# nomadkaraoke/python-audio-separator

Measured on AMD Instinct MI355X. Metric: audio-sec separated / wall-sec (RTF), UVR-MDX-NET 44.1kHz stereo, 1/2/4/8 GPU, higher is better.
Workload: dtype f32 (I/O and accumulators; matrix products on the 16-bit pipe from block-scaled two-part fp16 operands, 22-bit products -- see arithmetic; fp32-exact setting timed in arithmetic_ab)

## Files before the change

python-audio-separator_amd/csrc/asx.hip:

```cpp
#include <hip/hip_runtime.h>

#include <algorithm>
#include <atomic>
#include <cmath>
#include <cstdarg>
#include <cstdio>
#include <cstdlib>
#include <cstring>
#include <functional>
#include <map>
#include <string>
#include <mutex>
#include <vector>

#include "../../include/asx.h"
#include "knobs.h"
#include "resample_plan.h"
#include "flac_dec_plan.h"

static void grant_lds(const void *kernel, int bytes) {
  static std::mutex mu;
  static std::map<const void *, int> granted;
  std::lock_guard<std::mutex> lock(mu);
  int &g = granted[kernel];
// ... 24 lines not shown
#include "kernels_hd.h"
#include "kernels_vr.h"
#include "kernels_ens.h"
#include "kernels_resample.h"
#include "kernels_flac.h"
#include "kernels_pcm_encode.h"
#include "kernels_flac_dec.h"

using namespace asx;

#include "engine_core.h"
#include "engine_mdx.h"

static int opt_nonneg(int32_t v) { return v < 0 ? 0 : (int)v; }
static int opt_onoff(int32_t v) { return v > 0 ? 1 : 0; }

static const struct EngineOption {
  const char *key;
  int asx_engine::*field;
  int EngineKnobs::*knob;
  int (*norm)(int32_t);
  const char *refusal = nullptr;
  int shipped = 0;
} kOptions[] = {
    {"winograd", &asx_engine::winograd, &EngineKnobs::winograd, opt_nonneg,
     "asx_set_option: winograd = %d names a superseded kernel generation that only an experimental build carries "
     "(python build.py --experimental); this library has 0 (direct kernel) and 3 (the default)", 3},
    {"winograd_stationary", &asx_engine::winos, &EngineKnobs::winos, opt_nonneg,
     "asx_set_option: the weight-stationary Winograd kernel (measured slower) is in experimental builds only (python build.py --experimental)"},
    {"winograd_bf16x6", &asx_engine::wino6, &EngineKnobs::wino6, opt_nonneg},
    {"gemm_bf16x6", &asx_engine::gemm_bf16x6, &EngineKnobs::gemm_bf16x6, opt_onoff},
    {"gemm_f16x3", &asx_engine::gemm_f16x3, &EngineKnobs::gemm_f16x3, opt_onoff},
    {"conv_direct_f16x3", &asx_engine::conv3h, &EngineKnobs::conv3h, opt_nonneg},
    {"conv_fuse_input", &asx_engine::conv_fuse_input, &EngineKnobs::conv_fuse_input, opt_onoff},
    {"tdf_fuse_output", &asx_engine::tdf_fuse_output, &EngineKnobs::tdf_fuse_output, opt_onoff},
    {"conv3h_partial_scratch", &asx_engine::conv3h_ps, &EngineKnobs::conv3h_ps, opt_onoff},
    {"conv3h_walk", &asx_engine::conv3h_walk, &EngineKnobs::conv3h_walk, opt_onoff},
    {"conv3h_tiled", &asx_engine::conv3h_tiled, &EngineKnobs::conv3h_tiled, opt_onoff},
    {"conv3h_merge_out", &asx_engine::conv3h_merge, &EngineKnobs::conv3h_merge, opt_nonneg},
    {"conv_down_bf16x6", &asx_engine::down6, &EngineKnobs::down6, opt_onoff},
    {"conv_up_bf16x6", &asx_engine::up6, &EngineKnobs::up6, opt_onoff},
    {"gemm_pair_images", &asx_engine::pair_images, &EngineKnobs::pair_images, opt_onoff,
     "asx_set_option: gemm_pair_images = 1 needs an experimental build (python build.py --experimental): the pair-image reader measured no "
     "faster in the nets and is not in the default library"},
};

static const EngineOption *find_option(const char *fn, const char *key) {
  for (const EngineOption &o : kOptions)
    if (!strcmp(key, o.key)) return &o;
  set_err("%s: unknown option '%s'", fn, key);
  return nullptr;
}

extern "C" {
// ... 1414 lines not shown

int asx_op_conv(asx_engine *e, const char *op, const float *x_host, int32_t B, int32_t cin, int32_t t, int32_t f,
                const float *w_host, const float *b_host, int32_t cout, const float *aux_host, int32_t relu,
                float *y_host) {
  REQUIRE(e && op && x_host && w_host && y_host && B > 0 && cin > 0 && cout > 0 && t > 0 && f > 0,
          "asx_op_conv: bad argument");
  HIPCHK(hipSetDevice(e->device));
  int kind;
  int to = t, fo = f;
  ConvView view;
  if (!strcmp(op, "conv3x3")) kind = CK_3X3;
  else if (!strcmp(op, "conv3x3_to_tiled") || !strcmp(op, "conv3x3_tiled") || !strcmp(op, "conv3x3_from_tiled")) {
    kind = CK_3X3;
    view.x_tiled = strcmp(op, "conv3x3_to_tiled") != 0;
    view.y_tiled = strcmp(op, "conv3x3_from_tiled") != 0;
  } else if (!strcmp(op, "down")) {
    kind = CK_DOWN;
    to = t / 2;
    fo = f / 2;
  } else if (!strcmp(op, "conv1x1")) kind = CK_1X1;
  else if (!strcmp(op, "up")) {
    kind = CK_UP;
    to = 2 * t;
    fo = 2 * f;
    REQUIRE(aux_host, "asx_op_conv(up): skip tensor required");
  } else {
    set_err("asx_op_conv: unknown op '%s'", op);
    return ASX_ERR_INVALID;
  }
  ConvLayer L;
  DevBuf dx, dy, dskip;
  BufGuard g{{&dx, &dy, &dskip, &L.w, &L.b, &L.wu, &L.wu2, &L.wu3, &L.wus, &L.wu6, &L.wu6h, &L.w3h, &L.wd6, &L.wup6}};
  CHK(conv_setup(L, kind, cin, cout, relu ? 1 : 0));
  CHK(conv_pack(L, w_host, b_host, e->winograd));
  CHK(to_dev(dx, x_host, (size_t)B * cin * t * f));
  const size_t ny = (size_t)B * cout * to * fo;
  CHK(dy.ensure(ny * 4));
// ... 1231 lines not shown
}

int asx_counter(const asx_engine *e, const char *name, int64_t *out) {
  REQUIRE(e && name && out, "asx_counter: null argument");
  const std::string nm(name);
  if (nm == "tdf3_launches") *out = (int64_t)g_tdf3_launches.load();
  else if (nm == "tdf3h_launches") *out = (int64_t)g_tdf3h_launches.load();
  else if (nm == "attn6_launches") *out = (int64_t)g_attn6_launches.load();
  else if (nm == "attn6h_launches") *out = (int64_t)g_attn6h_launches.load();
  else if (nm == "tdf3_gather_launches") *out = (int64_t)g_tdf3_gather_launches.load();
  else if (nm == "wino6_launches") *out = (int64_t)g_wino6_launches.load();
  else if (nm == "wino6h_launches") *out = (int64_t)g_wino6h_launches.load();
  else if (nm == "conv3h_launches") *out = (int64_t)g_conv3h_launches.load();
  else if (nm == "conv3h_fin_launches") *out = (int64_t)g_conv3h_fin_launches.load();
  else if (nm == "conv3h_tiled_launches") *out = (int64_t)g_conv3h_tiled_launches.load();
  else if (nm == "conv3h_merged_dispatches") *out = (int64_t)g_conv3h_merged_dispatches.load();
  else if (nm == "tdf_fused_output_launches") *out = (int64_t)g_tdf_fused_output_launches.load();
  else if (nm == "tdf3_pair_image_launches") *out = (int64_t)g_tdf3ps_launches.load();
  else if (nm == "down6_launches") *out = (int64_t)g_down6_launches.load();
  else if (nm == "up6_launches") *out = (int64_t)g_up6_launches.load();
  else if (nm == "hd_rounds") *out = (int64_t)g_hd_rounds.load();
  else if (nm == "vr_net_passes") *out = (int64_t)g_vr_net_passes.load();
  else if (nm == "v3_net_passes") *out = (int64_t)g_v3_net_passes.load();
  else if (nm == "rof_net_passes") *out = (int64_t)g_rof_net_passes.load();
  else if (nm == "flac_block_cycles") *out = (int64_t)e->flac_block_cycles;
  else if (nm == "flac_crc16_cycles") *out = (int64_t)e->flac_crc16_cycles;
  else {
    set_err("asx_counter: unknown counter '%s'", name);
    return ASX_ERR_INVALID;
  }
  return ASX_OK;
}

int asx_debug_trace(uint64_t *host, int64_t n_u64) {
  REQUIRE(host && n_u64 > 0 && n_u64 <= 4096 * 8, "asx_debug_trace: bad argument");
// ... 263 lines not shown
```

python-audio-separator_amd/csrc/engine_core.h:

```cpp
#pragma once

static thread_local char g_err[512] = "";
static void set_err(const char *fmt, ...) {
  va_list ap;
  va_start(ap, fmt);
  vsnprintf(g_err, sizeof(g_err), fmt, ap);
  va_end(ap);
}
#define HIPCHK(x)                                                                       \
  do {                                                                                  \
    hipError_t e_ = (x);                                                                \
    if (e_ != hipSuccess) {                                                             \
      set_err("%s:%d %s -> %s", __FILE__, __LINE__, #x, hipGetErrorString(e_));         \
      return ASX_ERR_HIP;                                                               \
    }                                                                                   \
  } while (0)
#define CHK(x)                    \
  do {                            \
    int r_ = (x);                 \
    if (r_ != ASX_OK) return r_;  \
  } while (0)
#define REQUIRE(cond, ...)        \
  do {                            \
    if (!(cond)) {                \
// ... 191 lines not shown
  std::vector<RsTable *> rs_tabs;
  std::mutex rs_mu;
  hipEvent_t div_ev = nullptr;
  hipStream_t div_stream = nullptr;
  std::vector<DevBuf> skip;
  int winograd = 3;
  int winos = 0;
  int gemm_bf16x6 = 1;
  int gemm_f16x3 = 1;
  int wino6 = 144;
  int conv3h = 144;
  int conv3h_ps = 1;
  int conv3h_walk = 1;
  int conv3h_tiled = 1;
  int conv3h_merge = 144;
  int conv_fuse_input = 1;
  int tdf_fuse_output = 1;
  int down6 = 1;
  int up6 = 1;
  int pair_images = 0;
  std::vector<W3Entry> w3;
  std::mutex w3_mu;
  bool prof = false;
  int prof_nprod = 0;
  std::vector<ProfRec> recs;
};

static int pick_batch(const asx_engine *e) { return e->cfg.max_batch > 0 ? e->cfg.max_batch : 64; }

#include "batching.h"
// ... 75 lines not shown
```

python-audio-separator_amd/csrc/engine_mdx.h:

```cpp
#pragma once

template <class CFG>
static void launch_conv_t(const ConvArgs &a, int nblk, hipStream_t s) {
  grant_lds(&conv_mfma_kernel<CFG>, CFG::LDS_BYTES);
  hipLaunchKernelGGL(conv_mfma_kernel<CFG>, dim3(nblk), dim3(256), CFG::LDS_BYTES, s, a);
}

static int conv_tile_h(int kind) { return kind == CK_UP ? 4 : 8; }

static int pick_nrep_conv(int cout) {
  const int ct = (cout + 15) / 16;
  int best = 1, best_pad = 1 << 30;
  for (int n = 3; n >= 1; --n) {
    const int pad = ((ct + n - 1) / n) * n - ct;
    if (pad < best_pad) {
      best_pad = pad;
      best = n;
    }
  }
  return best;
}
static int pick_nrep_up(int cout) {
  const int ct = (cout + 15) / 16;
  if (knobs().up_nrep == 4 && (4 * ct) % 4 == 0) return 4;
// ... 188 lines not shown
  HIPCHK(hipMemcpy(L.b.p, bp.data(), bp.size() * 4, hipMemcpyHostToDevice));
  return ASX_OK;
}

template <class CFG>
static void launch_conv_dma_t(const ConvArgs &a, int nblk, hipStream_t s) {
  grant_lds(&conv_dma_kernel<CFG>, CFG::LDS_BYTES);
  hipLaunchKernelGGL(conv_dma_kernel<CFG>, dim3(nblk), dim3(256), CFG::LDS_BYTES, s, a);
}

static std::atomic<long long> g_wino6_launches{0};
static std::atomic<long long> g_wino6h_launches{0};
static std::atomic<long long> g_conv3h_launches{0};
static std::atomic<long long> g_conv3h_fin_launches{0};
static std::atomic<long long> g_conv3h_tiled_launches{0};
static std::atomic<long long> g_conv3h_merged_dispatches{0};
static std::atomic<long long> g_down6_launches{0};
static std::atomic<long long> g_up6_launches{0};

struct ConvView {
  int64_t x_bstride = 0;
  int64_t y_bstride = 0;
  const float *res = nullptr;
  int64_t aux_bstride = 0;
  int act = -1;
  float alpha = 1.f;
  const ConvLayer *fin = nullptr;
  const float *fin_x = nullptr;
  bool x_tiled = false, y_tiled = false;
};

static bool conv3h_takes(const asx_engine *e, const ConvLayer &L, bool dma, const float *res, int act, int T, int F, int64_t y_bstride, const float *y) {
#ifdef ASX_EXPERIMENTAL_KERNELS
  if (e->winos == 1 && L.wus.p != nullptr) return false;
#endif
  return L.kind == CK_3X3 && e->winograd == 3 && e->gemm_bf16x6 > 0 && e->gemm_f16x3 > 0 && e->conv3h > 0 && L.cin <= e->conv3h && L.w3h.p != nullptr && dma &&
         res == nullptr && (act == ACT_RELU || act == ACT_NONE) && F % 32 == 0 && (int64_t)Conv3hCfg::C * T * F < ((int64_t)1 << 29) &&
         y_bstride % 4 == 0 && (reinterpret_cast<uintptr_t>(y) & 15) == 0;
}

static bool conv3h_tiled_ok(const asx_engine *e, const ConvLayer &L, int T) { return T % 4 == 0 && (L.cin == Conv3hCfg::C || e->conv3h_ps > 0); }

static size_t conv3h_ps_need(const ConvLayer &L, int B, int T, int F) {
  if (L.kind != CK_3X3 || L.w3h.p == nullptr || L.cin <= Conv3hCfg::C || F % 32 != 0 || B <= 0 || T <= 0) return 0;
  return (size_t)(L.cin / Conv3hCfg::C) * (size_t)Conv3hCfg::ps_bytes(B, (T + 3) / 4, F / 32);
}

static const Conv3hWalkTab *conv3h_walk_find(const asx_engine *e, int B, int tilesT, int tilesF, int mode, int nob) {
  for (const Conv3hWalkTab *t : e->c3h_walks)
    if (t->B == B && t->tilesT == tilesT && t->tilesF == tilesF && t->mode == mode && t->nob == nob) return t;
  return nullptr;
}
static int conv3h_walk_ensure(asx_engine *e, const ConvLayer &L, int B, int T, int F) {
  if (L.kind != CK_3X3 || L.w3h.p == nullptr || F % 32 != 0 || B <= 0 || T <= 0) return ASX_OK;
  const int tilesT = (T + 3) / 4, tilesF = F / 32, nb = L.cin / Conv3hCfg::C;
  for (int k = 0; k < (nb > 1 ? 4 : 2); ++k) {
// ... 65 lines not shown
  a.aux_bstride = v.aux_bstride ? v.aux_bstride : (int64_t)L.cout * out_plane;
  const int th = conv_tile_h(L.kind);
  a.tilesT = (a.To + th - 1) / th;
  a.tilesF = (a.Fo + 63) / 64;
  const int nblk = a.CG * a.tilesT * a.tilesF * B;
  if (nblk <= 0) return ASX_OK;
  const double outpix = (double)B * a.To * a.Fo;
  const double flops = 2.0 * taps * L.cin * L.cout * outpix;
  double bytes = 4.0 * ((double)B * L.cin * T * F + (double)L.cout * outpix * (L.kind == CK_UP ? 4 : 1));
  if (L.kind == CK_UP && skip) bytes += 4.0 * (double)L.cout * outpix * 4;
  if (v.res) bytes += 4.0 * (double)L.cout * outpix;
  int bad = 0;
  const bool dma = (F % 4 == 0) && ((reinterpret_cast<uintptr_t>(v.fin ? v.fin_x : x) & 15) == 0) && (a.x_bstride % 4 == 0) && !knobs().no_dma;
  REQUIRE(!v.fin || (v.fin->w1f.p != nullptr && L.cin == Conv3hCfg::C && conv3h_takes(e, L, dma, v.res, a.act, T, F, a.y_bstride, y)),
          "fused-input 3x3 conv: the layer does not run conv3h_kernel");
  REQUIRE(!(v.x_tiled || v.y_tiled) || (conv3h_takes(e, L, dma, v.res, a.act, T, F, a.y_bstride, y) && conv3h_tiled_ok(e, L, T) && !(v.x_tiled && v.fin)),
          "tile-order 3x3 conv: the layer does not run conv3h_kernel in a form that has the layout");
  const ConvArgs &d = a;
#ifdef ASX_EXPERIMENTAL_KERNELS
  if (L.kind == CK_3X3 && e->winograd == 3 && e->winos == 1 && dma && L.wus.p != nullptr && a.Fo % 32 == 0 && v.res == nullptr &&
      (a.act == ACT_RELU || a.act == ACT_NONE) && (int64_t)L.cin * T * F < ((int64_t)1 << 30)) {
    ConvArgs wa = a;
    wa.wp = L.wus.f();
    wa.CG = L.wu_cg;
    wa.tilesF = a.Fo / 32;
    const int NS = (a.To + 1) / 2;
    const int base = wa.CG * wa.tilesF * B;
    int RB = std::max(1, std::min((NS + 7) / 8, (2048 + base - 1) / base));
    const int SPB = (NS + RB - 1) / RB;
    RB = (NS + SPB - 1) / SPB;
    wa.tilesT = RB;
// ... 40 lines not shown
        grant_lds(kern, Conv3hCfg::LDS_BYTES);
        hipLaunchKernelGGL(kern, dim3(256), dim3(512), Conv3hCfg::LDS_BYTES, s, ca);
      };
      if constexpr (FIN) {
        if (yt) one(&conv3h_kernel<0, false, true, 0, false, true>);
        else one(&conv3h_kernel<0, false, true>);
      } else if constexpr ((PS & 2) != 0) {
        if (v.x_tiled) one(&conv3h_kernel<0, false, false, PS, true, false>);
        else one(&conv3h_kernel<0, false, false, PS>);
      } else {
        if (v.x_tiled && yt) one(&conv3h_kernel<0, false, false, PS, true, true>);
        else if (v.x_tiled) one(&conv3h_kernel<0, false, false, PS, true, false>);
        else if (yt) one(&conv3h_kernel<0, false, false, PS, false, true>);
        else one(&conv3h_kernel<0, false, false, PS>);
      }
      if (v.x_tiled || yt) g_conv3h_tiled_launches.fetch_add(ca.nob);
    };
    const int64_t plane = (int64_t)T * F;
    const int64_t ps_item = Conv3hCfg::ps_item_bytes(tilesT, tilesF);
    REQUIRE(!ps || (ps_item < ((int64_t)1 << 32) && e->c3h_ps.p != nullptr && e->c3h_ps.bytes >= conv3h_ps_need(L, B, T, F)),
            "conv3h_kernel: the partial-sum scratch is not sized for %d x %d x %d (the workspace set-up sizes it)", B, T, F);
    Conv3hArgs walk{};
    walk.B = B;
    walk.T = T;
    walk.F = F;
    walk.x_bstride = a.x_bstride;
    walk.y_bstride = a.y_bstride;
    walk.tilesT = tilesT;
    walk.tilesF = tilesF;
    walk.bw = wt->bw;
    walk.walk = reinterpret_cast<const u32x4 *>(wt->tab.p);
// ... 121 lines not shown
  }
  if (L.kind == CK_3X3 && e->winograd == 1 && dma && L.wu.p != nullptr) {
    ConvArgs wa = a;
    wa.wp = L.wu.f();
    wa.CG = L.wu_cg;
    wa.NCI = L.wu_nci;
    wa.tilesT = (a.To + WinoCfg::TH - 1) / WinoCfg::TH;
    wa.tilesF = (a.Fo + WinoCfg::TW - 1) / WinoCfg::TW;
    const int nb = wa.CG * wa.tilesT * wa.tilesF * B;
    grant_lds(&conv_wino_kernel, WinoCfg::LDS_BYTES);
    return timed(e, cls, flops, bytes, s, [&]() {
      hipLaunchKernelGGL(conv_wino_kernel, dim3(nb), dim3(256), WinoCfg::LDS_BYTES, s, wa);
    });
  }
#endif
  if (L.kind == CK_DOWN && e->gemm_bf16x6 > 0 && e->down6 > 0 && L.wd6.p != nullptr && dma && (a.Fo & 3) == 0 && (reinterpret_cast<uintptr_t>(y) & 15) == 0 &&
      a.y_bstride % 4 == 0 && (v.res == nullptr || ((reinterpret_cast<uintptr_t>(v.res) & 15) == 0 && a.aux_bstride % 4 == 0))) {
    ConvArgs da = a;
    da.wp = reinterpret_cast<const float *>(L.wd6.p);
    da.CG = L.wd6_cg;
    da.NCI = L.wd6_nst;
    da.tilesT = (a.To + Down6Cfg::TH - 1) / Down6Cfg::TH;
    da.tilesF = (a.Fo + Down6Cfg::TW - 1) / Down6Cfg::TW;
    const int nb6 = da.CG * da.tilesT * da.tilesF * B;
    grant_lds(&conv_down6_kernel<3>, Down6CfgT<3>::LDS_BYTES);
    grant_lds(&conv_down6_kernel<6>, Down6CfgT<6>::LDS_BYTES);
    g_down6_launches.fetch_add(1);
    return timed(e, cls, flops, bytes, s, [&]() {
      e->prof_nprod = 6;
      if (L.wd6_nrep == 6) hipLaunchKernelGGL(conv_down6_kernel<6>, dim3(nb6), dim3(256), Down6CfgT<6>::LDS_BYTES, s, da);
      else hipLaunchKernelGGL(conv_down6_kernel<3>, dim3(nb6), dim3(256), Down6CfgT<3>::LDS_BYTES, s, da);
    });
  }
  if (L.kind == CK_UP && e->gemm_bf16x6 > 0 && e->up6 > 0 && L.wup6.p != nullptr && dma && (reinterpret_cast<uintptr_t>(y) & 15) == 0 && a.y_bstride % 4 == 0 &&
      (skip == nullptr || ((reinterpret_cast<uintptr_t>(skip) & 15) == 0 && a.aux_bstride % 4 == 0))) {
    ConvArgs ua = a;
    ua.wp = reinterpret_cast<const float *>(L.wup6.p);
    ua.CG = L.wup6_cg;
    ua.NCI = L.wup6_nst;
    ua.tilesT = (T + 1) / 2;
    ua.tilesF = (F + 63) / 64;
    const int nbu = ua.CG * ua.tilesT * ua.tilesF * B;
    grant_lds(&conv_up6_kernel<6>, Up6CfgT<6>::LDS_BYTES);
    grant_lds(&conv_up6_kernel<4>, Up6CfgT<4>::LDS_BYTES);
    grant_lds(&conv_up6_kernel<2>, Up6CfgT<2>::LDS_BYTES);
    g_up6_launches.fetch_add(1);
    return timed(e, cls, flops, bytes, s, [&]() {
      e->prof_nprod = 6;
      if (L.nrep == 6) hipLaunchKernelGGL(conv_up6_kernel<6>, dim3(nbu), dim3(256), Up6CfgT<6>::LDS_BYTES, s, ua);
      else if (L.nrep == 4) hipLaunchKernelGGL(conv_up6_kernel<4>, dim3(nbu), dim3(256), Up6CfgT<4>::LDS_BYTES, s, ua);
      else hipLaunchKernelGGL(conv_up6_kernel<2>, dim3(nbu), dim3(256), Up6CfgT<2>::LDS_BYTES, s, ua);
    });
  }
#define ASX_CONV_CASE(KH, KW, S, PAD, NR, KC, RPW, EPI)                                      \
  do {                                                                                       \
    if (dma) launch_conv_dma_t<ConvDmaCfg<KH, KW, S, PAD, NR, KC, RPW, EPI>>(d, nblk, s);    \
    else launch_conv_t<ConvCfg<KH, KW, S, PAD, NR, KC, RPW, EPI>>(a, nblk, s);               \
  } while (0)
  CHK(timed(e, cls, flops, bytes, s, [&]() {
    switch (L.kind) {
      case CK_3X3:
        if (L.nrep == 3 && L.kc == 4) ASX_CONV_CASE(3, 3, 1, 1, 3, 4, 2, EPI_BIAS_ACT);
        else if (L.nrep == 3) ASX_CONV_CASE(3, 3, 1, 1, 3, 8, 2, EPI_BIAS_ACT);
        else if (L.nrep == 2 && L.kc == 4) ASX_CONV_CASE(3, 3, 1, 1, 2, 4, 2, EPI_BIAS_ACT);
// ... 599 lines not shown
static int gn_launch(asx_engine *e, const float *x, int B, int C, int64_t P, const DevBuf &gw, const DevBuf &gb, const float *res,
                     const float *mul, float *y, hipStream_t s) {
  if (B <= 0) return ASX_OK;
  REQUIRE(C % 2 == 0 && gw.p && gb.p && e->gn_part.bytes >= (size_t)B * C * 16, "GroupNorm(2, %d): channels / workspace", C);
  double2 *part = reinterpret_cast<double2 *>(e->gn_part.p);
  const double bytes = 4.0 * (double)B * C * (double)P;
  CHK(timed(e, ASX_PROF_MISC, 0.0, bytes, s,
            [&]() { hipLaunchKernelGGL(gn_partial_kernel, dim3((unsigned)C, (unsigned)B), dim3(256), 0, s, x, C, P, part); }));
  const int nx = (int)std::max<int64_t>(1, std::min<int64_t>(32, (P / 4 + 1023) / 1024));
  return timed(e, ASX_PROF_MISC, 0.0, bytes * (2 + (res ? 1 : 0) + (mul ? 1 : 0)), s, [&]() {
    hipLaunchKernelGGL(gn_apply_kernel, dim3((unsigned)nx, (unsigned)C, (unsigned)B), dim3(256), 0, s, x, C, 2, P, part, gw.f(), gb.f(), 1e-5f, 1, res,
                       mul, y);
  });
}

static int block_forward(asx_engine *e, const Block &blk, float *&cur, float *dest, int B, hipStream_t s, const float *fin_x = nullptr,
                         TdfFusedOut *fo = nullptr) {
  auto next_free = [&](const float *a, const float *b) -> float * {
    for (int i = 0; i < 3; ++i)
      if (e->R[i].f() != a && e->R[i].f() != b) return e->R[i].f();
    return nullptr;
  };
  const bool gn = e->net.norm == 1;
  const int64_t plane = (int64_t)blk.t * blk.f;
  auto c3h = [&](size_t j, const float *xin) {
    const ConvLayer &L = blk.tfc[j];
    const bool dma = blk.f % 4 == 0 && (reinterpret_cast<uintptr_t>(xin) & 15) == 0 && !knobs().no_dma;
    return conv3h_takes(e, L, dma, nullptr, L.relu ? ACT_RELU : ACT_NONE, blk.t, blk.f, (int64_t)L.cout * plane, e->R[0].f()) && conv3h_tiled_ok(e, L, blk.t);
  };
  bool in_tiled = false;
  for (size_t j = 0; j < blk.tfc.size(); ++j) {
    float *out = next_free(cur, nullptr);
    ConvView v;
    if (j == 0 && fin_x) {
      v.fin = &e->first;
      v.fin_x = fin_x;
    }
    v.x_tiled = in_tiled;
    v.y_tiled = e->conv3h_tiled > 0 && !gn && j + 1 < blk.tfc.size() && (in_tiled || c3h(j, j == 0 && fin_x ? fin_x : cur)) && c3h(j + 1, out);
    in_tiled = v.y_tiled;
    CHK(conv_launch(e, blk.tfc[j], cur, nullptr, out, B, blk.t, blk.f, s, v));
    if (gn) CHK(gn_launch(e, out, B, blk.c, plane, blk.tfc[j].gn_w, blk.tfc[j].gn_b, nullptr, nullptr, out, s));
    cur = out;
  }
  const int64_t M = (int64_t)B * blk.c * blk.t;
  const int bnk = e->net.bn;
  if (bnk < 0) {
    if (dest) {
      HIPCHK(hipMemcpyAsync(dest, cur, (size_t)M * blk.f * 4, hipMemcpyDeviceToDevice, s));
      cur = dest;
    }
    return ASX_OK;
  }
// ... 32 lines not shown
  }
  const int T = e->net.dim_t, F = e->net.dim_f;
  const int n = e->net.num_blocks / 2;
  const bool gn = e->net.norm == 1;
  float *cur = e->R[0].f();
  const Block &blk0 = n > 0 ? e->enc[0] : e->mid;
  const bool fuse = e->conv_fuse_input > 0 && !gn && e->first.kind == CK_1X1 && e->first.cin == 4 && e->first.cout == Conv3hCfg::C && e->first.relu &&
                    e->first.w1f.p != nullptr && !blk0.tfc.empty() && blk0.tfc[0].cin == Conv3hCfg::C && blk0.tfc[0].cout == Conv3hCfg::C &&
                    conv3h_takes(e, blk0.tfc[0], F % 4 == 0 && (reinterpret_cast<uintptr_t>(spec_in) & 15) == 0 && !knobs().no_dma, nullptr,
                                 blk0.tfc[0].relu ? ACT_RELU : ACT_NONE, T, F, (int64_t)Conv3hCfg::C * T * F, e->R[1].f());
  if (!fuse) {
    CHK(conv_launch(e, e->first, spec_in, nullptr, cur, B, T, F, s));
    if (gn) CHK(gn_launch(e, cur, B, e->net.g, (int64_t)T * F, e->first.gn_w, e->first.gn_b, nullptr, nullptr, cur, s));
  }
  const float *fin_x = fuse ? spec_in : nullptr;
  for (int i = 0; i < n; ++i) {
    CHK(block_forward(e, e->enc[i], cur, e->skip[i].f(), B, s, i == 0 ? fin_x : nullptr));
    float *out = e->R[0].f();
    CHK(conv_launch(e, e->ds[i], cur, nullptr, out, B, e->enc[i].t, e->enc[i].f, s));
    if (gn)
      CHK(gn_launch(e, out, B, e->ds[i].cout, (int64_t)(e->enc[i].t / 2) * (e->enc[i].f / 2), e->ds[i].gn_w, e->ds[i].gn_b, nullptr, nullptr, out, s));
    cur = out;
  }
  TdfFusedOut fo{&e->final_, spec_out, false};
  const Block &last = n > 0 ? e->dec[n - 1] : e->mid;
  const bool try_fo = !gn && last.t == T && last.f == F;
  CHK(block_forward(e, e->mid, cur, nullptr, B, s, n == 0 ? fin_x : nullptr, n == 0 && try_fo ? &fo : nullptr));
  for (int i = 0; i < n; ++i) {
    const Block &blk = e->dec[i];
    float *out = nullptr;
    for (int r = 0; r < 3; ++r)
      if (e->R[r].f() != cur) {
        out = e->R[r].f();
        break;
      }
    CHK(conv_launch(e, e->us[i], cur, gn ? nullptr : e->skip[n - 1 - i].f(), out, B, blk.t / 2, blk.f / 2, s));
    if (gn)
      CHK(gn_launch(e, out, B, e->us[i].cout, (int64_t)blk.t * blk.f, e->us[i].gn_w, e->us[i].gn_b, nullptr, e->skip[n - 1 - i].f(), out, s));
    cur = out;
    CHK(block_forward(e, blk, cur, nullptr, B, s, nullptr, i == n - 1 && try_fo ? &fo : nullptr));
  }
  if (!fo.done) CHK(conv_launch(e, e->final_, cur, nullptr, spec_out, B, T, F, s));
  return ASX_OK;
}

static int net_walks_ensure(asx_engine *e, int Bn) {
  auto walks = [&](const Block &blk) -> int {
    for (const ConvLayer &L : blk.tfc) CHK(conv3h_walk_ensure(e, L, Bn, blk.t, blk.f));
    return ASX_OK;
  };
  for (const Block &blk : e->enc) CHK(walks(blk));
  CHK(walks(e->mid));
  for (const Block &blk : e->dec) CHK(walks(blk));
  return ASX_OK;
}
// ... 35 lines not shown
```

python-audio-separator_amd/csrc/kernels_updown6.h:

```cpp
#pragma once
#include "kernels_gemm3.h"

namespace asx {

template <int NREP_, int TH_ = 2>
struct Down6CfgT {
  static constexpr int TH = TH_, TW = 64, KC = 8, NREP = NREP_, NW = 16 * NREP_;
  static constexpr int IH = 2 * TH, IWA = 2 * TW;
  static constexpr int PLANE = IH * IWA;
  static constexpr int NJ = PLANE / 256;
  static constexpr int PAIRS = TH / 2;
  static constexpr int PS = PLANE + 16;
  static constexpr int XBYTES = KC * PS * 4;
  static constexpr int WSTAGE_U32 = 3 * NREP * 64 * 4;
  static constexpr int BUF = XBYTES + WSTAGE_U32 * 4;
  static constexpr int LDS_BYTES = BUF;
};
typedef Down6CfgT<3> Down6Cfg;

static inline uint16_t down6_bf16_rne(float v) {
  uint32_t u;
  memcpy(&u, &v, 4);
  if ((u & 0x7f800000u) == 0x7f800000u) return (uint16_t)((u >> 16) | ((u & 0xffffu) ? 0x40u : 0u));
  u += 0x7fffu + ((u >> 16) & 1u);
// ... 54 lines not shown
    for (int n = 0; n < NREP; ++n) acc[m][n] = ASX_MFMA_BF16(xh[m], bw[n], acc[m][n]);
  }
#pragma unroll
  for (int n = 0; n < NREP; ++n) bw[n] = __builtin_bit_cast(bf16x8, w_s[n * 64 + lane]);
#pragma unroll
  for (int m = 0; m < 2; ++m) {
#pragma unroll
    for (int n = 0; n < NREP; ++n) acc[m][n] = ASX_MFMA_BF16(xl[m], bw[n], acc[m][n]);
#pragma unroll
    for (int n = 0; n < NREP; ++n) acc[m][n] = ASX_MFMA_BF16(xm[m], bw[n], acc[m][n]);
#pragma unroll
    for (int n = 0; n < NREP; ++n) acc[m][n] = ASX_MFMA_BF16(xh[m], bw[n], acc[m][n]);
  }
}

template <int NREP, int TH = 2>
__global__ __launch_bounds__(256, TH == 2 ? 4 : 3) void conv_down6_kernel(ConvArgs a) {
  using C = Down6CfgT<NREP, TH>;
  extern __shared__ float lds_f[];
  char *lds = reinterpret_cast<char *>(lds_f);
  const int tid = threadIdx.x, lane = tid & 63;
  const int wave = __builtin_amdgcn_readfirstlane(tid >> 6);
  const int li = lane & 15, lk = lane >> 4;

  int lid = xcd_remap(blockIdx.x, gridDim.x);
  const int cg = lid % a.CG;
  lid /= a.CG;
  const int tf = lid % a.tilesF;
  lid /= a.tilesF;
  const int tt = lid % a.tilesT;
  const int b = lid / a.tilesT;
// ... 68 lines not shown
        split3_pair(c0d0.x, c0d0.y, hh[0], mm[0], ll[0]);
        split3_pair(c0d1.x, c0d1.y, hh[1], mm[1], ll[1]);
        split3_pair(c1d0.x, c1d0.y, hh[2], mm[2], ll[2]);
        split3_pair(c1d1.x, c1d1.y, hh[3], mm[3], ll[3]);
        xh[m] = __builtin_bit_cast(bf16x8, (u32x4){hh[0], hh[1], hh[2], hh[3]});
        xm[m] = __builtin_bit_cast(bf16x8, (u32x4){mm[0], mm[1], mm[2], mm[3]});
        xl[m] = __builtin_bit_cast(bf16x8, (u32x4){ll[0], ll[1], ll[2], ll[3]});
      }
      updown6_products<C::NREP>(w_s, lane, xh, xm, xl, acc[pi]);
    }
  }

  const int t = to0 + row;
  if (t >= a.To) return;
  float *yb = a.y + (int64_t)b * a.y_bstride;
  const float *rb = a.res ? a.res + (int64_t)b * a.aux_bstride : nullptr;
#pragma unroll
  for (int n = 0; n < C::NREP; ++n) {
    const int co = cg * C::NW + n * 16 + li;
    if (co >= a.Cout) continue;
    const float bv = a.bias[co];
#pragma unroll
    for (int pi = 0; pi < C::PAIRS; ++pi)
#pragma unroll
      for (int m = 0; m < 2; ++m) {
        const int col0 = TH == 2 ? (wave & 1) * 2 : 2 * pi;
        const int f = fo0 + (col0 + m) * 16 + lk * 4;
        const int64_t off = ((int64_t)co * a.To + t) * a.Fo + f;
        const f32x4 v = acc[pi][m][n];
        if ((a.Fo & 3) == 0 && f + 4 <= a.Fo) {
// ... 42 lines not shown
            const int c = st * C::KC + 2 * (lk + 4 * (kk >> 1)) + (kk & 1);
            const float v = (dy < 2 && co < cout && c < cin) ? w[(((size_t)c * cout + co) * 2 + dy) * 2 + dx] : 0.f;
            const uint16_t h = down6_bf16_rne(v);
            const float r1 = v - down6_bf16_f(h);
            const uint16_t m = down6_bf16_rne(r1);
            const uint16_t l = down6_bf16_rne(r1 - down6_bf16_f(m));
            const uint16_t parts[3] = {h, m, l};
            for (int p = 0; p < 3; ++p) o[((((size_t)(g * nst + st) * 3 + p) * NREP + n) * 64 + lane) * 8 + kk] = parts[p];
          }
        }
      }
  if (cg_out) *cg_out = cg;
  if (nst_out) *nst_out = nst;
}

template <int NREP>
__global__ __launch_bounds__(256, 4) void conv_up6_kernel(ConvArgs a) {
  using C = Up6CfgT<NREP>;
  static_assert(NREP % 2 == 0, "the dx tiles of a pair stay together");
  extern __shared__ float lds_f[];
  char *lds = reinterpret_cast<char *>(lds_f);
  const int tid = threadIdx.x, lane = tid & 63;
  const int wave = __builtin_amdgcn_readfirstlane(tid >> 6);
  const int li = lane & 15, lk = lane >> 4;

  int lid = xcd_remap(blockIdx.x, gridDim.x);
  const int cg = lid % a.CG;
  lid /= a.CG;
  const int tf = lid % a.tilesF;
  lid /= a.tilesF;
  const int tt = lid % a.tilesT;
// ... 85 lines not shown
      if (f >= a.F) continue;
      const int64_t off = ((int64_t)co * To2 + (2 * t + dy)) * Fo2 + 2 * f;
      const f32x4 v0 = acc[m][2 * np], v1 = acc[m][2 * np + 1];
      if (f + 4 <= a.F) {
        f32x4 r0, r1;
        r0.x = act_fn(v0.x + bv, a.act);
        r0.y = act_fn(v1.x + bv, a.act);
        r0.z = act_fn(v0.y + bv, a.act);
        r0.w = act_fn(v1.y + bv, a.act);
        r1.x = act_fn(v0.z + bv, a.act);
        r1.y = act_fn(v1.z + bv, a.act);
        r1.z = act_fn(v0.w + bv, a.act);
        r1.w = act_fn(v1.w + bv, a.act);
        r0 *= s0[m];
        r1 *= s1[m];
        *reinterpret_cast<f32x4 *>(yb + off) = r0;
        *reinterpret_cast<f32x4 *>(yb + off + 4) = r1;
      } else {
        const float o[8] = {v0.x, v1.x, v0.y, v1.y, v0.z, v1.z, v0.w, v1.w};
#pragma unroll
        for (int q = 0; q < 8; ++q)
          if (f + (q >> 1) < a.F) yb[off + q] = act_fn(o[q] + bv, a.act) * (sb != nullptr ? sb[off + q] : 1.f);
      }
    }
  }
}

}
```

python-audio-separator_amd/csrc/knobs.h:

```cpp
#pragma once

#include <algorithm>
#include <climits>
#include <cstdint>
#include <cstdlib>

#ifndef ASX_TDF2_DEFAULT
#define ASX_TDF2_DEFAULT 1
#endif

constexpr int HD_MAX_GROUPS = 6;

namespace knob {
inline bool set(const char *name) { return getenv(name) != nullptr; }
inline int num(const char *name, int def) { return set(name) ? atoi(getenv(name)) : def; }
inline int64_t num64(const char *name, int64_t def) { return set(name) ? atoll(getenv(name)) : def; }
inline double real(const char *name, double def) { return set(name) ? atof(getenv(name)) : def; }
inline bool on_unless_0(const char *name) { return !(set(name) && atoi(getenv(name)) == 0); }
inline bool off_unless_nonzero(const char *name) { return set(name) && atoi(getenv(name)) != 0; }
inline int clamped(const char *name, int def, int lo, int hi = INT_MAX) { return set(name) ? std::max(lo, std::min(hi, atoi(getenv(name)))) : def; }
}

struct Knobs {
  int poison = knob::num("ASX_POISON", -1);
// ... 71 lines not shown
#else
  int winograd = knob::num("ASX_WINOGRAD", 3) <= 0 ? 0 : 3;
  int winos = 0;
  int pair_images = 0;
#endif
  int gemm_bf16x6 = knob::num("ASX_GEMM_BF16X6", 1);
  int gemm_f16x3 = knob::num("ASX_GEMM_F16X3", 1);
  int wino6 = knob::clamped("ASX_WINO6", 144, 0);
  int conv3h = knob::clamped("ASX_CONV3H", 144, 0);
  int conv_fuse_input = 1;
  int tdf_fuse_output = 1;
  int conv3h_ps = 1;
  int conv3h_walk = 1;
  int conv3h_tiled = 1;
  int conv3h_merge = 144;
  int down6 = knob::num("ASX_DOWN6", 1);
  int up6 = knob::num("ASX_UP6", 1);
  bool fft3 = knob::on_unless_0("ASX_FFT3");
  bool fft3p = knob::on_unless_0("ASX_FFT3P");
};
```

python-audio-separator_amd/engine.py:

```python
from __future__ import annotations

import ctypes as C
import os
from dataclasses import dataclass

import numpy as np

_HERE = os.path.dirname(os.path.abspath(__file__))

ASX_FLAG_MATCH_MIX = 1
PROF_CLASSES = ["stft", "conv3x3", "tdf", "down", "up", "conv1x1", "istft", "ola", "finalize", "misc"]


class AsxError(RuntimeError):
    pass


def lib_path() -> str:
    return os.path.join(_HERE, "libasx.so")


class _MdxCfg(C.Structure):
    _fields_ = [("n_fft", C.c_int32), ("hop_length", C.c_int32), ("dim_f", C.c_int32), ("segment_size", C.c_int32),
                ("overlap", C.c_double), ("enable_denoise", C.c_int32), ("max_batch", C.c_int32), ("win_length", C.c_int32),
# ... 1455 lines not shown
        spec = _f32(spec)
        out = np.empty_like(spec)
        self._check(self._lib.asx_net_forward(self._h, _ptr(spec), spec.shape[0], _ptr(out)))
        return out

    def run_model(self, wave: np.ndarray, is_match_mix: bool = False) -> np.ndarray:
        wave = _f32(wave)
        out = np.empty_like(wave)
        self._check(self._lib.asx_run_model(self._h, _ptr(wave), wave.shape[0], _ptr(out),
                                            ASX_FLAG_MATCH_MIX if is_match_mix else 0))
        return out

    def op_conv(self, op: str, x, w, b, aux=None, relu=True) -> np.ndarray:
        x, w, b = _f32(x), _f32(w), _f32(b)
        B, cin, t, f = x.shape
        if op == "up":
            cout = w.shape[1]
            shape = (B, cout, 2 * t, 2 * f)
        elif op == "down":
            cout = w.shape[0]
            shape = (B, cout, t // 2, f // 2)
        else:
            cout = w.shape[0]
            shape = (B, cout, t, f)
        aux = _f32(aux) if aux is not None else None
        y = np.empty(shape, np.float32)
        self._check(self._lib.asx_op_conv(self._h, op.encode(), _ptr(x), B, cin, t, f, _ptr(w), _ptr(b), cout,
                                          _optptr(aux), int(relu), _ptr(y)))
        return y

    def op_tdf(self, x, w, bias, scale, shift, res=None) -> np.ndarray:
        x, w, scale, shift = _f32(x), _f32(w), _f32(scale), _f32(shift)
        B, c, t, k = x.shape
        n = w.shape[0]
# ... 172 lines not shown
```

Before: 1767.

## Have down/up level-change convs write tile-order output for the next conv3h

Result: no change. 1784 (median of 6 runs) (+1.0%).

```diff
diff --git a/python-audio-separator_amd/csrc/asx.hip b/python-audio-separator_amd/csrc/asx.hip
--- a/python-audio-separator_amd/csrc/asx.hip
+++ b/python-audio-separator_amd/csrc/asx.hip
@@ -62,6 +62,7 @@
 
 static int opt_nonneg(int32_t v) { return v < 0 ? 0 : (int)v; }
 static int opt_onoff(int32_t v) { return v > 0 ? 1 : 0; }
+static int opt_bits2(int32_t v) { return v < 0 ? 0 : (int)(v & 3); }
 
 static const struct EngineOption {
   const char *key;
@@ -86,6 +87,7 @@
     {"conv3h_walk", &asx_engine::conv3h_walk, &EngineKnobs::conv3h_walk, opt_onoff},
     {"conv3h_tiled", &asx_engine::conv3h_tiled, &EngineKnobs::conv3h_tiled, opt_onoff},
     {"conv3h_merge_out", &asx_engine::conv3h_merge, &EngineKnobs::conv3h_merge, opt_nonneg},
+    {"updown_tiled", &asx_engine::updown_tiled, &EngineKnobs::updown_tiled, opt_bits2},
     {"conv_down_bf16x6", &asx_engine::down6, &EngineKnobs::down6, opt_onoff},
     {"conv_up_bf16x6", &asx_engine::up6, &EngineKnobs::up6, opt_onoff},
     {"gemm_pair_images", &asx_engine::pair_images, &EngineKnobs::pair_images, opt_onoff,
@@ -1530,13 +1532,15 @@
     kind = CK_3X3;
     view.x_tiled = strcmp(op, "conv3x3_to_tiled") != 0;
     view.y_tiled = strcmp(op, "conv3x3_from_tiled") != 0;
-  } else if (!strcmp(op, "down")) {
+  } else if (!strcmp(op, "down") || !strcmp(op, "down_to_tiled")) {
     kind = CK_DOWN;
     to = t / 2;
     fo = f / 2;
+    view.y_tiled = strcmp(op, "down") != 0;
   } else if (!strcmp(op, "conv1x1")) kind = CK_1X1;
-  else if (!strcmp(op, "up")) {
+  else if (!strcmp(op, "up") || !strcmp(op, "up_to_tiled")) {
     kind = CK_UP;
+    view.y_tiled = strcmp(op, "up") != 0;
     to = 2 * t;
     fo = 2 * f;
     REQUIRE(aux_host, "asx_op_conv(up): skip tensor required");
@@ -2798,11 +2802,14 @@
   else if (nm == "conv3h_launches") *out = (int64_t)g_conv3h_launches.load();
   else if (nm == "conv3h_fin_launches") *out = (int64_t)g_conv3h_fin_launches.load();
   else if (nm == "conv3h_tiled_launches") *out = (int64_t)g_conv3h_tiled_launches.load();
+  else if (nm == "conv3h_lvl_input_launches") *out = (int64_t)g_conv3h_lvl_input_launches.load();
   else if (nm == "conv3h_merged_dispatches") *out = (int64_t)g_conv3h_merged_dispatches.load();
   else if (nm == "tdf_fused_output_launches") *out = (int64_t)g_tdf_fused_output_launches.load();
   else if (nm == "tdf3_pair_image_launches") *out = (int64_t)g_tdf3ps_launches.load();
   else if (nm == "down6_launches") *out = (int64_t)g_down6_launches.load();
   else if (nm == "up6_launches") *out = (int64_t)g_up6_launches.load();
+  else if (nm == "down6_tiled_launches") *out = (int64_t)g_down6_tiled_launches.load();
+  else if (nm == "up6_tiled_launches") *out = (int64_t)g_up6_tiled_launches.load();
   else if (nm == "hd_rounds") *out = (int64_t)g_hd_rounds.load();
   else if (nm == "vr_net_passes") *out = (int64_t)g_vr_net_passes.load();
   else if (nm == "v3_net_passes") *out = (int64_t)g_v3_net_passes.load();
diff --git a/python-audio-separator_amd/csrc/engine_core.h b/python-audio-separator_amd/csrc/engine_core.h
--- a/python-audio-separator_amd/csrc/engine_core.h
+++ b/python-audio-separator_amd/csrc/engine_core.h
@@ -229,6 +229,7 @@
   int conv3h_walk = 1;
   int conv3h_tiled = 1;
   int conv3h_merge = 144;
+  int updown_tiled = 3;
   int conv_fuse_input = 1;
   int tdf_fuse_output = 1;
   int down6 = 1;
diff --git a/python-audio-separator_amd/csrc/engine_mdx.h b/python-audio-separator_amd/csrc/engine_mdx.h
--- a/python-audio-separator_amd/csrc/engine_mdx.h
+++ b/python-audio-separator_amd/csrc/engine_mdx.h
@@ -226,9 +226,13 @@
 static std::atomic<long long> g_conv3h_launches{0};
 static std::atomic<long long> g_conv3h_fin_launches{0};
 static std::atomic<long long> g_conv3h_tiled_launches{0};
+static std::atomic<long long> g_conv3h_lvl_input_launches{0};
 static std::atomic<long long> g_conv3h_merged_dispatches{0};
 static std::atomic<long long> g_down6_launches{0};
 static std::atomic<long long> g_up6_launches{0};
+static std::atomic<long long> g_down6_tiled_launches{0};
+static std::atomic<long long> g_up6_tiled_launches{0};
+static constexpr int UP6_YT = 1;
 
 struct ConvView {
   int64_t x_bstride = 0;
@@ -240,6 +244,7 @@
   const ConvLayer *fin = nullptr;
   const float *fin_x = nullptr;
   bool x_tiled = false, y_tiled = false;
+  bool x_lvl = false;
 };
 
 static bool conv3h_takes(const asx_engine *e, const ConvLayer &L, bool dma, const float *res, int act, int T, int F, int64_t y_bstride, const float *y) {
@@ -252,6 +257,17 @@
 }
 
 static bool conv3h_tiled_ok(const asx_engine *e, const ConvLayer &L, int T) { return T % 4 == 0 && (L.cin == Conv3hCfg::C || e->conv3h_ps > 0); }
+
+static bool updown6_takes(const asx_engine *e, const ConvLayer &L, bool dma, const float *aux, int64_t aux_bstride, int Fo, int64_t y_bstride, const float *y) {
+  if (!(e->gemm_bf16x6 > 0 && dma && (reinterpret_cast<uintptr_t>(y) & 15) == 0 && y_bstride % 4 == 0 &&
+        (aux == nullptr || ((reinterpret_cast<uintptr_t>(aux) & 15) == 0 && aux_bstride % 4 == 0))))
+    return false;
+  if (L.kind == CK_DOWN) return e->down6 > 0 && L.wd6.p != nullptr && (Fo & 3) == 0;
+  return L.kind == CK_UP && e->up6 > 0 && L.wup6.p != nullptr;
+}
+static bool updown6_tiled_ok(const ConvLayer &L, const float *res, int To, int Fo) {
+  return res == nullptr && L.cout % Conv3hCfg::C == 0 && To % 4 == 0 && Fo % 32 == 0 && (int64_t)Conv3hCfg::C * To * Fo < ((int64_t)1 << 29);
+}
 
 static size_t conv3h_ps_need(const ConvLayer &L, int B, int T, int F) {
   if (L.kind != CK_3X3 || L.w3h.p == nullptr || L.cin <= Conv3hCfg::C || F % 32 != 0 || B <= 0 || T <= 0) return 0;
@@ -347,7 +363,12 @@
   const bool dma = (F % 4 == 0) && ((reinterpret_cast<uintptr_t>(v.fin ? v.fin_x : x) & 15) == 0) && (a.x_bstride % 4 == 0) && !knobs().no_dma;
   REQUIRE(!v.fin || (v.fin->w1f.p != nullptr && L.cin == Conv3hCfg::C && conv3h_takes(e, L, dma, v.res, a.act, T, F, a.y_bstride, y)),
           "fused-input 3x3 conv: the layer does not run conv3h_kernel");
-  REQUIRE(!(v.x_tiled || v.y_tiled) || (conv3h_takes(e, L, dma, v.res, a.act, T, F, a.y_bstride, y) && conv3h_tiled_ok(e, L, T) && !(v.x_tiled && v.fin)),
+  const bool lvl = L.kind == CK_DOWN || L.kind == CK_UP;
+  const int To2 = L.kind == CK_UP ? 2 * T : a.To, Fo2 = L.kind == CK_UP ? 2 * F : a.Fo;
+  REQUIRE(!lvl || !(v.x_tiled || v.y_tiled) ||
+              (!v.x_tiled && updown6_takes(e, L, dma, L.kind == CK_UP ? skip : v.res, a.aux_bstride, a.Fo, a.y_bstride, y) && updown6_tiled_ok(L, v.res, To2, Fo2)),
+          "tile-order level-change conv: the layer does not run the bf16 x 6 kernel on whole tiles");
+  REQUIRE(lvl || !(v.x_tiled || v.y_tiled) || (conv3h_takes(e, L, dma, v.res, a.act, T, F, a.y_bstride, y) && conv3h_tiled_ok(e, L, T) && !(v.x_tiled && v.fin)),
           "tile-order 3x3 conv: the layer does not run conv3h_kernel in a form that has the layout");
   const ConvArgs &d = a;
 #ifdef ASX_EXPERIMENTAL_KERNELS
@@ -418,7 +439,8 @@
         else if (yt) one(&conv3h_kernel<0, false, false, PS, false, true>);
         else one(&conv3h_kernel<0, false, false, PS>);
       }
-      if (v.x_tiled || yt) g_conv3h_tiled_launches.fetch_add(ca.nob);
+      if (v.x_tiled && v.x_lvl) g_conv3h_lvl_input_launches.fetch_add(ca.nob);
+      if ((v.x_tiled && !v.x_lvl) || yt) g_conv3h_tiled_launches.fetch_add(ca.nob);
     };
     const int64_t plane = (int64_t)T * F;
     const int64_t ps_item = Conv3hCfg::ps_item_bytes(tilesT, tilesF);
@@ -570,8 +592,7 @@
     });
   }
 #endif
-  if (L.kind == CK_DOWN && e->gemm_bf16x6 > 0 && e->down6 > 0 && L.wd6.p != nullptr && dma && (a.Fo & 3) == 0 && (reinterpret_cast<uintptr_t>(y) & 15) == 0 &&
-      a.y_bstride % 4 == 0 && (v.res == nullptr || ((reinterpret_cast<uintptr_t>(v.res) & 15) == 0 && a.aux_bstride % 4 == 0))) {
+  if (L.kind == CK_DOWN && updown6_takes(e, L, dma, v.res, a.aux_bstride, a.Fo, a.y_bstride, y)) {
     ConvArgs da = a;
     da.wp = reinterpret_cast<const float *>(L.wd6.p);
     da.CG = L.wd6_cg;
@@ -581,15 +602,19 @@
     const int nb6 = da.CG * da.tilesT * da.tilesF * B;
     grant_lds(&conv_down6_kernel<3>, Down6CfgT<3>::LDS_BYTES);
     grant_lds(&conv_down6_kernel<6>, Down6CfgT<6>::LDS_BYTES);
+    grant_lds(&conv_down6_kernel<3, 2, true>, Down6CfgT<3>::LDS_BYTES);
+    grant_lds(&conv_down6_kernel<6, 2, true>, Down6CfgT<6>::LDS_BYTES);
     g_down6_launches.fetch_add(1);
+    if (v.y_tiled) g_down6_tiled_launches.fetch_add(1);
     return timed(e, cls, flops, bytes, s, [&]() {
       e->prof_nprod = 6;
-      if (L.wd6_nrep == 6) hipLaunchKernelGGL(conv_down6_kernel<6>, dim3(nb6), dim3(256), Down6CfgT<6>::LDS_BYTES, s, da);
+      if (v.y_tiled && L.wd6_nrep == 6) hipLaunchKernelGGL((conv_down6_kernel<6, 2, true>), dim3(nb6), dim3(256), Down6CfgT<6>::LDS_BYTES, s, da);
+      else if (v.y_tiled) hipLaunchKernelGGL((conv_down6_kernel<3, 2, true>), dim3(nb6), dim3(256), Down6CfgT<3>::LDS_BYTES, s, da);
+      else if (L.wd6_nrep == 6) hipLaunchKernelGGL(conv_down6_kernel<6>, dim3(nb6), dim3(256), Down6CfgT<6>::LDS_BYTES, s, da);
       else hipLaunchKernelGGL(conv_down6_kernel<3>, dim3(nb6), dim3(256), Down6CfgT<3>::LDS_BYTES, s, da);
     });
   }
-  if (L.kind == CK_UP && e->gemm_bf16x6 > 0 && e->up6 > 0 && L.wup6.p != nullptr && dma && (reinterpret_cast<uintptr_t>(y) & 15) == 0 && a.y_bstride % 4 == 0 &&
-      (skip == nullptr || ((reinterpret_cast<uintptr_t>(skip) & 15) == 0 && a.aux_bstride % 4 == 0))) {
+  if (L.kind == CK_UP && updown6_takes(e, L, dma, skip, a.aux_bstride, a.Fo, a.y_bstride, y)) {
     ConvArgs ua = a;
     ua.wp = reinterpret_cast<const float *>(L.wup6.p);
     ua.CG = L.wup6_cg;
@@ -600,10 +625,15 @@
     grant_lds(&conv_up6_kernel<6>, Up6CfgT<6>::LDS_BYTES);
     grant_lds(&conv_up6_kernel<4>, Up6CfgT<4>::LDS_BYTES);
     grant_lds(&conv_up6_kernel<2>, Up6CfgT<2>::LDS_BYTES);
+    grant_lds(&conv_up6_kernel<6, UP6_YT>, Up6CfgT<6>::LDS_BYTES);
+    grant_lds(&conv_up6_kernel<4, UP6_YT>, Up6CfgT<4>::LDS_BYTES);
     g_up6_launches.fetch_add(1);
+    if (v.y_tiled) g_up6_tiled_launches.fetch_add(1);
     return timed(e, cls, flops, bytes, s, [&]() {
       e->prof_nprod = 6;
-      if (L.nrep == 6) hipLaunchKernelGGL(conv_up6_kernel<6>, dim3(nbu), dim3(256), Up6CfgT<6>::LDS_BYTES, s, ua);
+      if (v.y_tiled && L.nrep == 6) hipLaunchKernelGGL((conv_up6_kernel<6, UP6_YT>), dim3(nbu), dim3(256), Up6CfgT<6>::LDS_BYTES, s, ua);
+      else if (v.y_tiled) hipLaunchKernelGGL((conv_up6_kernel<4, UP6_YT>), dim3(nbu), dim3(256), Up6CfgT<4>::LDS_BYTES, s, ua);
+      else if (L.nrep == 6) hipLaunchKernelGGL(conv_up6_kernel<6>, dim3(nbu), dim3(256), Up6CfgT<6>::LDS_BYTES, s, ua);
       else if (L.nrep == 4) hipLaunchKernelGGL(conv_up6_kernel<4>, dim3(nbu), dim3(256), Up6CfgT<4>::LDS_BYTES, s, ua);
       else hipLaunchKernelGGL(conv_up6_kernel<2>, dim3(nbu), dim3(256), Up6CfgT<2>::LDS_BYTES, s, ua);
     });
@@ -1233,8 +1263,15 @@
   });
 }
 
+static bool block_conv3h_tiled(const asx_engine *e, const Block &blk, size_t j, const float *xin) {
+  if (j >= blk.tfc.size()) return false;
+  const ConvLayer &L = blk.tfc[j];
+  const bool dma = blk.f % 4 == 0 && (reinterpret_cast<uintptr_t>(xin) & 15) == 0 && !knobs().no_dma;
+  return conv3h_takes(e, L, dma, nullptr, L.relu ? ACT_RELU : ACT_NONE, blk.t, blk.f, (int64_t)L.cout * blk.t * blk.f, e->R[0].f()) && conv3h_tiled_ok(e, L, blk.t);
+}
+
 static int block_forward(asx_engine *e, const Block &blk, float *&cur, float *dest, int B, hipStream_t s, const float *fin_x = nullptr,
-                         TdfFusedOut *fo = nullptr) {
+                         TdfFusedOut *fo = nullptr, bool in_tiled = false) {
   auto next_free = [&](const float *a, const float *b) -> float * {
     for (int i = 0; i < 3; ++i)
       if (e->R[i].f() != a && e->R[i].f() != b) return e->R[i].f();
@@ -1242,12 +1279,7 @@
   };
   const bool gn = e->net.norm == 1;
   const int64_t plane = (int64_t)blk.t * blk.f;
-  auto c3h = [&](size_t j, const float *xin) {
-    const ConvLayer &L = blk.tfc[j];
-    const bool dma = blk.f % 4 == 0 && (reinterpret_cast<uintptr_t>(xin) & 15) == 0 && !knobs().no_dma;
-    return conv3h_takes(e, L, dma, nullptr, L.relu ? ACT_RELU : ACT_NONE, blk.t, blk.f, (int64_t)L.cout * plane, e->R[0].f()) && conv3h_tiled_ok(e, L, blk.t);
-  };
-  bool in_tiled = false;
+  auto c3h = [&](size_t j, const float *xin) { return block_conv3h_tiled(e, blk, j, xin); };
   for (size_t j = 0; j < blk.tfc.size(); ++j) {
     float *out = next_free(cur, nullptr);
     ConvView v;
@@ -1256,6 +1288,7 @@
       v.fin_x = fin_x;
     }
     v.x_tiled = in_tiled;
+    v.x_lvl = j == 0 && in_tiled;
     v.y_tiled = e->conv3h_tiled > 0 && !gn && j + 1 < blk.tfc.size() && (in_tiled || c3h(j, j == 0 && fin_x ? fin_x : cur)) && c3h(j + 1, out);
     in_tiled = v.y_tiled;
     CHK(conv_launch(e, blk.tfc[j], cur, nullptr, out, B, blk.t, blk.f, s, v));
@@ -1318,10 +1351,19 @@
     if (gn) CHK(gn_launch(e, cur, B, e->net.g, (int64_t)T * F, e->first.gn_w, e->first.gn_b, nullptr, nullptr, cur, s));
   }
   const float *fin_x = fuse ? spec_in : nullptr;
+  auto lvl_tiled = [&](int bit, const ConvLayer &L, const Block &reader, const float *x, int Fin, const float *aux, const float *y, int To, int Fo) {
+    const bool dma = Fin % 4 == 0 && (reinterpret_cast<uintptr_t>(x) & 15) == 0 && !knobs().no_dma;
+    return (e->updown_tiled & bit) != 0 && !gn && L.cout == reader.c && To == reader.t && Fo == reader.f && !reader.tfc.empty() && reader.tfc[0].cin == L.cout &&
+           updown6_takes(e, L, dma, aux, (int64_t)L.cout * reader.t * reader.f, reader.f, (int64_t)L.cout * reader.t * reader.f, y) &&
+           updown6_tiled_ok(L, nullptr, reader.t, reader.f) && block_conv3h_tiled(e, reader, 0, y);
+  };
+  bool in_tiled = false;
   for (int i = 0; i < n; ++i) {
-    CHK(block_forward(e, e->enc[i], cur, e->skip[i].f(), B, s, i == 0 ? fin_x : nullptr));
+    CHK(block_forward(e, e->enc[i], cur, e->skip[i].f(), B, s, i == 0 ? fin_x : nullptr, nullptr, in_tiled));
     float *out = e->R[0].f();
-    CHK(conv_launch(e, e->ds[i], cur, nullptr, out, B, e->enc[i].t, e->enc[i].f, s));
+    ConvView dv;
+    dv.y_tiled = in_tiled = lvl_tiled(1, e->ds[i], i + 1 < n ? e->enc[i + 1] : e->mid, cur, e->enc[i].f, nullptr, out, e->enc[i].t / 2, e->enc[i].f / 2);
+    CHK(conv_launch(e, e->ds[i], cur, nullptr, out, B, e->enc[i].t, e->enc[i].f, s, dv));
     if (gn)
       CHK(gn_launch(e, out, B, e->ds[i].cout, (int64_t)(e->enc[i].t / 2) * (e->enc[i].f / 2), e->ds[i].gn_w, e->ds[i].gn_b, nullptr, nullptr, out, s));
     cur = out;
@@ -1329,7 +1371,7 @@
   TdfFusedOut fo{&e->final_, spec_out, false};
   const Block &last = n > 0 ? e->dec[n - 1] : e->mid;
   const bool try_fo = !gn && last.t == T && last.f == F;
-  CHK(block_forward(e, e->mid, cur, nullptr, B, s, n == 0 ? fin_x : nullptr, n == 0 && try_fo ? &fo : nullptr));
+  CHK(block_forward(e, e->mid, cur, nullptr, B, s, n == 0 ? fin_x : nullptr, n == 0 && try_fo ? &fo : nullptr, in_tiled));
   for (int i = 0; i < n; ++i) {
     const Block &blk = e->dec[i];
     float *out = nullptr;
@@ -1338,11 +1380,13 @@
         out = e->R[r].f();
         break;
       }
-    CHK(conv_launch(e, e->us[i], cur, gn ? nullptr : e->skip[n - 1 - i].f(), out, B, blk.t / 2, blk.f / 2, s));
+    ConvView uv;
+    uv.y_tiled = in_tiled = lvl_tiled(2, e->us[i], blk, cur, blk.f / 2, e->skip[n - 1 - i].f(), out, 2 * (blk.t / 2), 2 * (blk.f / 2));
+    CHK(conv_launch(e, e->us[i], cur, gn ? nullptr : e->skip[n - 1 - i].f(), out, B, blk.t / 2, blk.f / 2, s, uv));
     if (gn)
       CHK(gn_launch(e, out, B, e->us[i].cout, (int64_t)blk.t * blk.f, e->us[i].gn_w, e->us[i].gn_b, nullptr, e->skip[n - 1 - i].f(), out, s));
     cur = out;
-    CHK(block_forward(e, blk, cur, nullptr, B, s, nullptr, i == n - 1 && try_fo ? &fo : nullptr));
+    CHK(block_forward(e, blk, cur, nullptr, B, s, nullptr, i == n - 1 && try_fo ? &fo : nullptr, in_tiled));
   }
   if (!fo.done) CHK(conv_launch(e, e->final_, cur, nullptr, spec_out, B, T, F, s));
   return ASX_OK;
diff --git a/python-audio-separator_amd/csrc/kernels_updown6.h b/python-audio-separator_amd/csrc/kernels_updown6.h
--- a/python-audio-separator_amd/csrc/kernels_updown6.h
+++ b/python-audio-separator_amd/csrc/kernels_updown6.h
@@ -1,7 +1,24 @@
 #pragma once
+#include "kernels_conv3h.h"
 #include "kernels_gemm3.h"
 
 namespace asx {
+
+struct UpDown6Tl {
+  static constexpr int64_t slice_off(int To, int Fo, int ctile) { return (int64_t)(ctile / 3) * Conv3hCfg::tl_item_bytes(To, Fo); }
+  static constexpr int64_t down_store(int To, int Fo, int t, int ftile, int ctile, int lane) {
+    return slice_off(To, Fo, ctile) + Conv3hCfg::tl_block_off(Fo, t, ftile, ctile % 3) + Conv3hCfg::tl_store_lane(lane);
+  }
+  static constexpr int64_t up_piece(int To, int Fo, int t, int span, int ctile, int lane, int r) {
+    return slice_off(To, Fo, ctile) + Conv3hCfg::tl_block_off(Fo, t, 2 * span + (lane >> 5), ctile % 3) + Conv3hCfg::tl_in_block(2 * ((lane >> 4) & 1) + r, lane & 15);
+  }
+  static constexpr int up_xchg_reg(int lane, int p) { return ((lane >> 5) ^ p) & 1; }
+  static constexpr int up_xchg_src(int lane, int p) { return ((((((lane >> 4) & 1) << 1) | (lane >> 5)) ^ (2 * p)) << 4) | (lane & 15); }
+  static constexpr int up_xchg_store(int lane, int p) { return ((lane >> 4) ^ p) & 1; }
+  static constexpr int64_t up_store(int To, int Fo, int t, int span, int ctile, int lane, int s) {
+    return slice_off(To, Fo, ctile) + Conv3hCfg::tl_block_off(Fo, t, 2 * span + s, ctile % 3) + Conv3hCfg::tl_store_lane(lane);
+  }
+};
 
 template <int NREP_, int TH_ = 2>
 struct Down6CfgT {
@@ -92,7 +109,7 @@
   }
 }
 
-template <int NREP, int TH = 2>
+template <int NREP, int TH = 2, bool YT = false>
 __global__ __launch_bounds__(256, TH == 2 ? 4 : 3) void conv_down6_kernel(ConvArgs a) {
   using C = Down6CfgT<NREP, TH>;
   extern __shared__ float lds_f[];
@@ -191,6 +208,30 @@
   const int t = to0 + row;
   if (t >= a.To) return;
   float *yb = a.y + (int64_t)b * a.y_bstride;
+  if constexpr (YT) {
+    char *yt = reinterpret_cast<char *>(yb);
+#pragma unroll
+    for (int n = 0; n < C::NREP; ++n) {
+      const int ctile = cg * C::NREP + n;
+      if (ctile * 16 >= a.Cout) continue;
+      const float bv = a.bias[ctile * 16 + li];
+#pragma unroll
+      for (int pi = 0; pi < C::PAIRS; ++pi)
+#pragma unroll
+        for (int m = 0; m < 2; ++m) {
+          const int ftile = fo0 / 16 + (TH == 2 ? (wave & 1) * 2 : 2 * pi) + m;
+          if (ftile * 16 >= a.Fo) continue;
+          const f32x4 v = acc[pi][m][n];
+          f32x4 o;
+          o.x = act_fn(v.x + bv, a.act);
+          o.y = act_fn(v.y + bv, a.act);
+          o.z = act_fn(v.z + bv, a.act);
+          o.w = act_fn(v.w + bv, a.act);
+          *reinterpret_cast<f32x4 *>(yt + UpDown6Tl::down_store(a.To, a.Fo, t, ftile, ctile, lane)) = o;
+        }
+    }
+    return;
+  }
   const float *rb = a.res ? a.res + (int64_t)b * a.aux_bstride : nullptr;
 #pragma unroll
   for (int n = 0; n < C::NREP; ++n) {
@@ -263,7 +304,7 @@
   if (nst_out) *nst_out = nst;
 }
 
-template <int NREP>
+template <int NREP, int YT = 0>
 __global__ __launch_bounds__(256, 4) void conv_up6_kernel(ConvArgs a) {
   using C = Up6CfgT<NREP>;
   static_assert(NREP % 2 == 0, "the dx tiles of a pair stay together");
@@ -379,8 +420,40 @@
         r1.w = act_fn(v1.w + bv, a.act);
         r0 *= s0[m];
         r1 *= s1[m];
-        *reinterpret_cast<f32x4 *>(yb + off) = r0;
-        *reinterpret_cast<f32x4 *>(yb + off + 4) = r1;
+        if constexpr (YT == 1) {
+          char *yt = reinterpret_cast<char *>(yb);
+          const int span = fo0 / 16 + col0 + m;
+          *reinterpret_cast<f32x4 *>(yt + UpDown6Tl::up_piece(To2, Fo2, 2 * t + dy, span, ct, lane, 0)) = r0;
+          *reinterpret_cast<f32x4 *>(yt + UpDown6Tl::up_piece(To2, Fo2, 2 * t + dy, span, ct, lane, 1)) = r1;
+        } else if constexpr (YT == 2) {
+          char *yt = reinterpret_cast<char *>(yb);
+          const int span = fo0 / 16 + col0 + m;
+          f32x4 st[2];
+#pragma unroll
+          for (int p = 0; p < 2; ++p) {
+            const u32x4 offer = __builtin_bit_cast(u32x4, UpDown6Tl::up_xchg_reg(lane, p) ? r1 : r0);
+            const int src = UpDown6Tl::up_xchg_src(lane, p) * 4;
+            u32x4 took;
+            took.x = (unsigned)__builtin_amdgcn_ds_bpermute(src, (int)offer.x);
+            took.y = (unsigned)__builtin_amdgcn_ds_bpermute(src, (int)offer.y);
+            took.z = (unsigned)__builtin_amdgcn_ds_bpermute(src, (int)offer.z);
+            took.w = (unsigned)__builtin_amdgcn_ds_bpermute(src, (int)offer.w);
+            const f32x4 got = __builtin_bit_cast(f32x4, took);
+            const bool first = UpDown6Tl::up_xchg_store(lane, p) == 0;
+            if (p == 0) {
+              st[0] = got;
+              st[1] = got;
+            } else {
+              st[0] = first ? got : st[0];
+              st[1] = first ? st[1] : got;
+            }
+          }
+#pragma unroll
+          for (int k = 0; k < 2; ++k) *reinterpret_cast<f32x4 *>(yt + UpDown6Tl::up_store(To2, Fo2, 2 * t + dy, span, ct, lane, k)) = st[k];
+        } else {
+          *reinterpret_cast<f32x4 *>(yb + off) = r0;
+          *reinterpret_cast<f32x4 *>(yb + off + 4) = r1;
+        }
       } else {
         const float o[8] = {v0.x, v1.x, v0.y, v1.y, v0.z, v1.z, v0.w, v1.w};
 #pragma unroll
diff --git a/python-audio-separator_amd/csrc/knobs.h b/python-audio-separator_amd/csrc/knobs.h
--- a/python-audio-separator_amd/csrc/knobs.h
+++ b/python-audio-separator_amd/csrc/knobs.h
@@ -109,6 +109,7 @@
   int conv3h_walk = 1;
   int conv3h_tiled = 1;
   int conv3h_merge = 144;
+  int updown_tiled = 3;
   int down6 = knob::num("ASX_DOWN6", 1);
   int up6 = knob::num("ASX_UP6", 1);
   bool fft3 = knob::on_unless_0("ASX_FFT3");
diff --git a/python-audio-separator_amd/engine.py b/python-audio-separator_amd/engine.py
--- a/python-audio-separator_amd/engine.py
+++ b/python-audio-separator_amd/engine.py
@@ -1493,10 +1493,10 @@
     def op_conv(self, op: str, x, w, b, aux=None, relu=True) -> np.ndarray:
         x, w, b = _f32(x), _f32(w), _f32(b)
         B, cin, t, f = x.shape
-        if op == "up":
+        if op in ("up", "up_to_tiled"):
             cout = w.shape[1]
             shape = (B, cout, 2 * t, 2 * f)
-        elif op == "down":
+        elif op in ("down", "down_to_tiled"):
             cout = w.shape[0]
             shape = (B, cout, t // 2, f // 2)
         else:
```
